# XuShenLZ/conflict_rez

Hardware: AMD Instinct MI355X
Metric: OBCA MPC-step solves/sec (4 vehicles, N=30) (higher is better)
Workload: dtype f64

## Files before the change

### conflict_rez_amd/csrc/cfz_engine.hip

```cpp

#include <hip/hip_runtime.h>
#include <stdio.h>
#include <string.h>

#include <algorithm>
#include <cstdio>
#include <cstdlib>
#include <unistd.h>
#include <cmath>
#include <string>
#include <tuple>
#include <vector>

#include "../../include/confrez_hip.h"
#include "cfz_solver.inl"
#include "cfz_audit.inl"
#include "cfz_disturb.inl"
#include "cfz_comm.inl"
#include "cfz_common.h"

thread_local std::string cfz_g_err;

namespace {

// ... 53 lines not shown
__global__ void loop_prep(int S, int V, int N, int T, const double *ref_table, const int32_t *table_of, const int32_t *kidx,
                          const double *pred, const double *state, double *x0, double *ref, double *nbr,
                          double *zu, int r, const int32_t *xperm, const int32_t *xrank, cfz::DisturbArgs dz, int step, cfz::CommArgs cm) {
  const long tid = (long)blockIdx.x * blockDim.x + threadIdx.x;
  if (tid >= (long)(xperm ? S : S * V) * N) return;
  const int k = (int)(tid % N);
  int b = (int)(tid / N);
  if (xperm) b = b * V + xperm[b * V + r];
  const int s = b / V, v = b - s * V;
  if (k < 5) x0[b * 5 + k] = dz.sigma ? cfz::disturb_add(state[b * 5 + k], cfz::disturb_value(dz, s, v, step, k)) : state[b * 5 + k];
  prep_stage(b, k, N, T, V, v, ref_table + ((size_t)table_of[s] * V + v) * T * 7, kidx[s], pred + (size_t)b * 7 * N,
             pred + (size_t)s * V * 7 * N, 7, xrank ? xrank + (size_t)s * V : nullptr, r, cm, s, step, ref, nbr, zu);
}

__global__ void advance_clock(int S, int K, int32_t *kidx) {
  const int s = blockIdx.x * blockDim.x + threadIdx.x;
  if (s < S) kidx[s] += K;
}

__global__ void loop_post(int S, int V, int N, const KArgs *ka, const int32_t *status, const int32_t *iters, const double *zu,
                          double *pred, double *state, int32_t *kidx, double *rec, int32_t *rec_si, int r, const int32_t *xperm,
                          cfz::DisturbArgs dz, int step, int32_t *carry, double *msg, const KArgs *pool, const int32_t *problem_of) {
  int b = blockIdx.x * blockDim.x + threadIdx.x;
  if (b >= (xperm ? S : S * V)) return;
  if (xperm) b = b * V + xperm[b * V + r];
  double *pb = pred + (size_t)b * 7 * N;
  if (status[b] == 0) {
    for (int i = 0; i < 7 * N; ++i) pb[i] = zu[(size_t)b * 7 * N + i];
  } else {
    for (int c = 0; c < 7; ++c)
      for (int k = 0; k + 1 < N; ++k) pb[c * N + k] = pb[c * N + k + 1];
  }
  if (msg)
    for (int i = 0; i < 7 * N; ++i) msg[(size_t)b * 7 * N + i] = pb[i];
  double z[5], out[5];
  for (int i = 0; i < 5; ++i) z[i] = state[b * 5 + i];
  double a0 = pb[5 * N], w0 = pb[6 * N];
  const int s = b / V, v = b - s * V;
  const cfz::KSpec &sp = (pool ? pool + problem_of[s] : ka)->sp;
  if (dz.sigma) {
    a0 = cfz::disturb_clip(cfz::disturb_add(a0, cfz::disturb_value(dz, s, v, step, 5)), sp.bounds[8], sp.bounds[9]);
    w0 = cfz::disturb_clip(cfz::disturb_add(w0, cfz::disturb_value(dz, s, v, step, 6)), sp.bounds[10], sp.bounds[11]);
  }
  cfz::rk4_step<false>(z, a0, w0, sp.dt, sp.wb, kPlantSubsteps, out, nullptr);
  if (dz.sigma)
    for (int i = 0; i < 5; ++i) out[i] = cfz::disturb_add(out[i], cfz::disturb_value(dz, s, v, step, 7 + i));
  for (int i = 0; i < 5; ++i) state[b * 5 + i] = out[i];
  if (kidx && (xperm ? r == V - 1 : b % V == 0)) kidx[b / V] += 1;
  if (carry) carry[b] = status[b] == 0;
  if (rec) {
    double *r = rec + (size_t)b * 7;
    for (int i = 0; i < 5; ++i) r[i] = out[i];
    r[5] = a0; r[6] = w0;
    rec_si[b] = status[b]; rec_si[S * V + b] = iters[b];
  }
}

__global__ void vs_prep(int S, int V, int n_own, int N, int T, const int32_t *own, const double *table, const int32_t *k0, int t,
                        const double *allpred, const double *pred, const double *state, double *x0, double *ref, double *nbr,
                        double *zu) {
  const long tid = (long)blockIdx.x * blockDim.x + threadIdx.x;
  if (tid >= (long)S * n_own * N) return;
  const int k = (int)(tid % N);
  const int b = (int)(tid / N);
  const int s = b / n_own, o = b - s * n_own;
  if (k < 5) x0[b * 5 + k] = state[b * 5 + k];
  prep_stage(b, k, N, T, V, own[o], table + (size_t)o * T * 7, k0[s] + t, pred + (size_t)b * 7 * N, allpred + (size_t)s * V * 3 * N, 3,
             nullptr, 0, cfz::comm_none(), s, t, ref, nbr, zu);
}

__global__ __launch_bounds__(1024) void order_by_iters(int B, const int32_t *iters, int32_t *order) {
  __shared__ int hist[1024];
  const int t = threadIdx.x;
  hist[t] = 0;
  __syncthreads();
  for (int b = t; b < B; b += 1024) atomicAdd(&hist[1023 - min(iters[b], 1023)], 1);
  __syncthreads();
  if (t == 0) { int acc = 0; for (int i = 0; i < 1024; ++i) { const int c = hist[i]; hist[i] = acc; acc += c; } }
  __syncthreads();
  for (int b = t; b < B; b += 1024) order[atomicAdd(&hist[1023 - min(iters[b], 1023)], 1)] = b;
}

#ifdef CFZ_LOOP_TRACE
constexpr int kLoopTraceWords = 5;
__device__ long long *cfz_loop_trace_buf;
#define CFZ_MARK(c) do { if (threadIdx.x == 0) __hip_atomic_store(&ctrl[4 + blockIdx.x], (c), __ATOMIC_RELAXED, __HIP_MEMORY_SCOPE_AGENT); } while (0)
#define CFZ_ITEM_STAMP(w, flag) do { if (threadIdx.x == 0) { long long *cfz_r = cfz_loop_trace_buf + ((size_t)t * B + b) * kLoopTraceWords;      \
                                                        cfz_r[w] = (long long)wall_clock64(); if ((w) == 0) cfz_r[4] = 1 + (flag); } } while (0)
#else
#define CFZ_MARK(c) do { } while (0)
#define CFZ_ITEM_STAMP(w, flag) do { } while (0)
#endif
#define CFZ_LOOP_ARGS const KArgs *__restrict__ ka, int S, int V, int K, int T, const double *ref_table, const int32_t *table_of,        \
                      const int32_t *kidx0, int t_base, double *pred, double *state, double *scratch, int32_t *qbuf, int32_t *ctrl,       \
                      int32_t *done, int32_t *status, int32_t *iters, double *stats, int32_t *iter_sum, double *wst, int wst_stride,     \
                      int prio_lag, int prio_tail, double *rec, int32_t *rec_si
__global__ __launch_bounds__(cfz::kNL, CFZ_WAVES_PER_SIMD) void loop_kernel(CFZ_LOOP_ARGS) {
  constexpr bool kSeq = false, kDist = false, kComm = false, kPool = false;
  const KArgs *const pool = nullptr; const int32_t *const problem_of = nullptr; constexpr bool dz_clip = true;
  const cfz::CommArgs cm = cfz::comm_none();
  const int32_t *const xperm = nullptr, *const xrank = nullptr;
  const cfz::DisturbArgs dz = cfz::disturb_none();
  const int step0 = 0;
#include "cfz_loop_body.inl"
}

__global__ __launch_bounds__(cfz::kNL, CFZ_WAVES_PER_SIMD) void loop_kernel_seq(CFZ_LOOP_ARGS, const int32_t *xperm, const int32_t *xrank) {
  constexpr bool kSeq = true, kDist = false, kComm = false, kPool = false;
  const KArgs *const pool = nullptr; const int32_t *const problem_of = nullptr; constexpr bool dz_clip = true;
  const cfz::CommArgs cm = cfz::comm_none();
  const cfz::DisturbArgs dz = cfz::disturb_none();
  const int step0 = 0;
#include "cfz_loop_body.inl"
}

__global__ __launch_bounds__(cfz::kNL, CFZ_WAVES_PER_SIMD) void loop_kernel_dist(CFZ_LOOP_ARGS, cfz::DisturbArgs dz, int step0) {
  constexpr bool kSeq = false, kDist = true, kComm = false, kPool = false;
  const KArgs *const pool = nullptr; const int32_t *const problem_of = nullptr; constexpr bool dz_clip = true;
  const cfz::CommArgs cm = cfz::comm_none();
  const int32_t *const xperm = nullptr, *const xrank = nullptr;
#include "cfz_loop_body.inl"
}

__global__ __launch_bounds__(cfz::kNL, CFZ_WAVES_PER_SIMD) void loop_kernel_seq_dist(CFZ_LOOP_ARGS, const int32_t *xperm,
                                                                 const int32_t *xrank, cfz::DisturbArgs dz, int step0) {
  constexpr bool kSeq = true, kDist = true, kComm = false, kPool = false;
  const KArgs *const pool = nullptr; const int32_t *const problem_of = nullptr; constexpr bool dz_clip = true;
  const cfz::CommArgs cm = cfz::comm_none();
#include "cfz_loop_body.inl"
}

__global__ __launch_bounds__(cfz::kNL, CFZ_WAVES_PER_SIMD) void loop_kernel_comm(CFZ_LOOP_ARGS, cfz::DisturbArgs dz, int step0,
                                                             cfz::CommArgs cm) {
  constexpr bool kSeq = false, kDist = true, kComm = true, kPool = false;
  const KArgs *const pool = nullptr; const int32_t *const problem_of = nullptr; constexpr bool dz_clip = true;
  const int32_t *const xperm = nullptr, *const xrank = nullptr;
#include "cfz_loop_body.inl"
}

__global__ __launch_bounds__(cfz::kNL, CFZ_WAVES_PER_SIMD) void loop_kernel_seq_comm(CFZ_LOOP_ARGS, const int32_t *xperm,
                                                                 const int32_t *xrank, cfz::DisturbArgs dz, int step0, cfz::CommArgs cm) {
  constexpr bool kSeq = true, kDist = true, kComm = true, kPool = false;
  const KArgs *const pool = nullptr; const int32_t *const problem_of = nullptr; constexpr bool dz_clip = true;
#include "cfz_loop_body.inl"
}

__global__ __launch_bounds__(cfz::kNL, CFZ_WAVES_PER_SIMD) void loop_kernel_pool(CFZ_LOOP_ARGS, cfz::DisturbArgs dz, int step0,
                                                             const KArgs *__restrict__ pool, const int32_t *__restrict__ problem_of, int dz_clip) {
  constexpr bool kSeq = false, kDist = true, kComm = false, kPool = true;
  const cfz::CommArgs cm = cfz::comm_none();
  const int32_t *const xperm = nullptr, *const xrank = nullptr;
#include "cfz_loop_body.inl"
}

__global__ __launch_bounds__(cfz::kNL, CFZ_WAVES_PER_SIMD) void loop_kernel_seq_pool(CFZ_LOOP_ARGS, const int32_t *xperm, const int32_t *xrank,
                                                                 cfz::DisturbArgs dz, int step0, const KArgs *__restrict__ pool,
                                                                 const int32_t *__restrict__ problem_of, int dz_clip) {
  constexpr bool kSeq = true, kDist = true, kComm = false, kPool = true;
  const cfz::CommArgs cm = cfz::comm_none();
#include "cfz_loop_body.inl"
}

__global__ __launch_bounds__(cfz::kNL, CFZ_WAVES_PER_SIMD) void loop_kernel_pool_comm(CFZ_LOOP_ARGS, cfz::DisturbArgs dz, int step0, cfz::CommArgs cm,
                                                                  const KArgs *__restrict__ pool, const int32_t *__restrict__ problem_of, int dz_clip) {
  constexpr bool kSeq = false, kDist = true, kComm = true, kPool = true;
  const int32_t *const xperm = nullptr, *const xrank = nullptr;
#include "cfz_loop_body.inl"
}

__global__ __launch_bounds__(cfz::kNL, CFZ_WAVES_PER_SIMD) void loop_kernel_seq_pool_comm(CFZ_LOOP_ARGS, const int32_t *xperm, const int32_t *xrank,
                                                                      cfz::DisturbArgs dz, int step0, cfz::CommArgs cm,
                                                                      const KArgs *__restrict__ pool, const int32_t *__restrict__ problem_of, int dz_clip) {
  constexpr bool kSeq = true, kDist = true, kComm = true, kPool = true;
#include "cfz_loop_body.inl"
}
#undef CFZ_LOOP_ARGS

constexpr int kLoopPrioLag = 0, kLoopPrioTailDiv = 0;
#ifdef CFZ_LOOP_TRACE
long long *g_loop_trace_dev = nullptr; size_t g_loop_trace_items = 0; int g_loop_trace_grid = 0;
#endif
struct LoopVariant { const void *fn; bool seq, dist, comm, pool; };
const LoopVariant kLoopVariants[10] = {
    {(const void *)loop_kernel, false, false, false, false},          {(const void *)loop_kernel_seq, true, false, false, false},
    {(const void *)loop_kernel_dist, false, true, false, false},      {(const void *)loop_kernel_seq_dist, true, true, false, false},
    {(const void *)loop_kernel_comm, false, true, true, false},       {(const void *)loop_kernel_seq_comm, true, true, true, false},
    {(const void *)loop_kernel_pool, false, true, false, true},       {(const void *)loop_kernel_seq_pool, true, true, false, true},
    {(const void *)loop_kernel_pool_comm, false, true, true, true},   {(const void *)loop_kernel_seq_pool_comm, true, true, true, true}};

int loop_variant(bool seq, bool dz_on, bool cm_on, bool pb_on) {
  const bool dist = dz_on || cm_on || pb_on;
  for (int i = 0; i < 10; ++i) {
    const LoopVariant &v = kLoopVariants[i];
    if (v.seq == seq && v.dist == dist && v.comm == cm_on && v.pool == pb_on) return i;
  }
  return -1;
}

__global__ void comm_fill(cfz::CommArgs cm, int S, int V, int tau0, long n, int32_t *delivered) {
  const long i = (long)blockIdx.x * blockDim.x + threadIdx.x;
  if (i >= n) return;
  const int u = (int)(i % V), v = (int)((i / V) % V), s = (int)((i / ((long)V * V)) % S), k = (int)(i / ((long)V * V * S));
  delivered[i] = u == v ? 1 : (cfz::comm_delivered(cm.seed, cm.stream[s], v, u, tau0 + k, cm.p_drop[s]) ? 1 : 0);
}

__global__ void disturb_fill(cfz::DisturbArgs dz, int S, int V, int t0, long n, double *d) {
  const long i = (long)blockIdx.x * blockDim.x + threadIdx.x;
  if (i >= n) return;
  const int c = (int)(i % cfz::kDisturbN);
  const long b = i / cfz::kDisturbN;
  const int v = (int)(b % V), s = (int)((b / V) % S), k = (int)(b / ((long)V * S));
  d[i] = cfz::disturb_value(dz, s, v, t0 + k, c);
}

__device__ inline void point_segment(double qx, double qy, double ax, double ay, double bx, double by, double &dist2, double &nx, double &ny) {
  const double ex = bx - ax, ey = by - ay, wx = qx - ax, wy = qy - ay;
  double t = (wx * ex + wy * ey) / (ex * ex + ey * ey);
  t = fmin(fmax(t, 0.0), 1.0);
  nx = wx - t * ex; ny = wy - t * ey;
  dist2 = nx * nx + ny * ny;
}

__device__ inline bool polygon_gap(const double PV[4][2], const double QV[4][2], double &nx, double &ny, double &dist) {
  double best = INFINITY, bx = 0.0, by = 0.0;
  for (int v = 0; v < 4; ++v)
    for (int e = 0; e < 4; ++e) {
      double d2, ux, uy;
      point_segment(QV[v][0], QV[v][1], PV[e][0], PV[e][1], PV[(e + 1) & 3][0], PV[(e + 1) & 3][1], d2, ux, uy);
      if (d2 < best) { best = d2; bx = ux; by = uy; }
      point_segment(PV[v][0], PV[v][1], QV[e][0], QV[e][1], QV[(e + 1) & 3][0], QV[(e + 1) & 3][1], d2, ux, uy);
      if (d2 < best) { best = d2; bx = -ux; by = -uy; }
    }
  dist = sqrt(best);
  if (!(dist > 1e-12)) return false;
  nx = bx / dist; ny = by / dist;
  return true;
}

__device__ inline void cone_duals(const double A[4][2], const double b[4], const double V[4][2], double nx, double ny, double lam[4]) {
  int v = 0; double sup = -INFINITY;
  for (int i = 0; i < 4; ++i) { const double h = nx * V[i][0] + ny * V[i][1]; if (h > sup) { sup = h; v = i; } }
  int i0 = 0, i1 = 1; double r0 = INFINITY, r1 = INFINITY;
  for (int i = 0; i < 4; ++i) {
    const double r = fabs(A[i][0] * V[v][0] + A[i][1] * V[v][1] - b[i]);
    if (r < r0) { r1 = r0; i1 = i0; r0 = r; i0 = i; } else if (r < r1) { r1 = r; i1 = i; }
  }
  const int ia = i0 < i1 ? i0 : i1, ib = i0 < i1 ? i1 : i0;
  const double det = A[ia][0] * A[ib][1] - A[ib][0] * A[ia][1];
  for (int i = 0; i < 4; ++i) lam[i] = 0.0;
  lam[ia] = fmax((A[ib][1] * nx - A[ib][0] * ny) / det, 0.0);
  lam[ib] = fmax((-A[ia][1] * nx + A[ia][0] * ny) / det, 0.0);
}

__global__ void dual_ws_kernel(const cfz::KSpec sp, int n, const double *poses, double *l, double *mu_out, double *d) {
  const int tid = blockIdx.x * blockDim.x + threadIdx.x;
  const int no = sp.n_obs;
  if (tid >= n * no) return;
  const int k = tid / no, j = tid - k * no;
  double A[4][2], b[4], V[4][2];
  for (int i = 0; i < 4; ++i) {
    A[i][0] = sp.A_obs[j][i][0]; A[i][1] = sp.A_obs[j][i][1]; b[i] = sp.b_obs[j][i];
// ... 97 lines not shown
  if (i >= n) return;
  double s, c;
  sincos(traj[i * 7 + 2], &s, &c);
  cs[i * 2] = c; cs[i * 2 + 1] = s;
}

__global__ __launch_bounds__(64) void audit_kernel(const KArgs *__restrict__ ka, int K, int S, int V, const double *traj,
                                                   const double *cs, const double *goal, const cfz::AuditPoly *obs_in, double il0, double il1,
                                                   double pos_tol, double psi_tol, double v_tol, double *clear, int32_t *where,
                                                   int32_t *first_contact, int32_t *arrive) {
  __shared__ cfz::AuditPoly obs[cfz::kMaxObs];
  const int s = blockIdx.x, lane = threadIdx.x;
  const int no = ka->sp.n_obs;
  if (lane < no) obs[lane] = obs_in[lane];
  double g[4];
  for (int i = 0; i < 4; ++i) g[i] = ka->sp.g[i];
  const double il[2] = {il0, il1};
  __syncthreads();
  cfz::AuditAcc acc;
  cfz::audit_lane(acc, lane, 64, K, V, traj + (size_t)s * V * 7, (long)S * V * 7, goal + (size_t)s * V * 3, cs + (size_t)s * V * 2, no,
                  obs, g, il, pos_tol, psi_tol, v_tol);
  for (int off = 32; off > 0; off >>= 1) {
    cfz::AuditAcc o;
    o.vv = __shfl_xor(acc.vv, off, 64); o.vv_t = __shfl_xor(acc.vv_t, off, 64); o.vv_u = __shfl_xor(acc.vv_u, off, 64);
    o.vv_w = __shfl_xor(acc.vv_w, off, 64);
    o.vo = __shfl_xor(acc.vo, off, 64); o.vo_t = __shfl_xor(acc.vo_t, off, 64); o.vo_v = __shfl_xor(acc.vo_v, off, 64);
    o.vo_j = __shfl_xor(acc.vo_j, off, 64);
    o.first = __shfl_xor(acc.first, off, 64);
    for (int v = 0; v < cfz::kAuditMaxV; ++v) o.arrive[v] = __shfl_xor(acc.arrive[v], off, 64);
    cfz::audit_merge(acc, o);
  }
  if (lane == 0) cfz::audit_store(acc, V, clear + (size_t)s * 2, where + (size_t)s * 6, first_contact + s, arrive + (size_t)s * V);
}

}

struct cfz_handle {
  int device = 0, max_batch = 0;
  cfz::KSpec ks;
  cfz::Lay lay;
  cfz_spec spec0;
  cfz_options opt0;
  size_t lds_bytes = 0;
  int blocks_per_cu = 0;
  hipStream_t stream = nullptr;
  hipEvent_t ev0 = nullptr, ev1 = nullptr;
  float last_ms = 0.f;
  double *obs_tab = nullptr;
  KArgs *kargs = nullptr;
  double *wst = nullptr;
  int32_t *carry = nullptr, *slots = nullptr;
  int32_t *stage_host = nullptr;
  hipEvent_t ev_stage = nullptr;
  int wst_stride = 0, carry_duals = 1;
  bool carry_set = false, slots_set = false, ms_pending = false;
  const int32_t *carry_ext = nullptr;
  double *x0 = nullptr, *ref = nullptr, *nbr = nullptr, *zu = nullptr, *stats = nullptr;
  int32_t *status = nullptr, *iters = nullptr;
  double *l = nullptr, *m = nullptr, *lam_ij = nullptr, *lam_ji = nullptr, *s = nullptr;
  struct Loop {
    int S = 0, T = 0, P = 0;
    double *ref_table = nullptr, *pred = nullptr, *state = nullptr;
    int32_t *kidx = nullptr, *order = nullptr, *table_of = nullptr;
    bool have_order = false;
    int32_t *xperm = nullptr, *xrank = nullptr, *xlist = nullptr;
    std::vector<int32_t> xperm_host;
    double *rec = nullptr;
    int32_t *rec_si = nullptr;
    int rec_cap = 0, rec_used = 0;
    void *dz_buf = nullptr, *dz_zero = nullptr;
    uint64_t dz_seed = 0;
    bool dz_on = false;
    void *cm_buf = nullptr;
    double *cm_ring = nullptr;
    uint64_t cm_seed = 0;
    int cm_max_age = 0, cm_compensate = 0, cm_tau_on = 0, cm_ring_slots = 0;
    bool cm_on = false;
    KArgs *pb_pool = nullptr;
    int32_t *pb_of = nullptr;
    int pb_cap = 0;
    bool pb_on = false;
    double *pred2 = nullptr, *scratch = nullptr;
    int32_t *queue = nullptr, *ctrl = nullptr, *done = nullptr, *iter_sum = nullptr;
    int queue_cap = 0, grid_blocks = 0, steps_done = 0;
  } lp;
  long last_iter_sum = 0, last_converged = 0, last_status[6] = {0, 0, 0, 0, 0, 0};
  CfzArena arena;
};

namespace {

int launch_solve(cfz_handle *h, int B, const double *x0, const double *ref, const double *nbr, double *zu,
                 int32_t *status, int32_t *iters, double *stats, bool duals, hipStream_t st,
                 const int32_t *order = nullptr, int carry_all = 0, int grid = 0, bool pool = false) {
  DualPtrs du = {nullptr, nullptr, nullptr, nullptr, nullptr};
  if (duals) du = {h->l, h->m, h->lam_ij, h->lam_ji, h->s};
  if ((h->carry_set || h->slots_set) && st != h->stream) HIP_OK(hipStreamWaitEvent(st, h->ev_stage, 0));
  HIP_OK(hipEventRecord(h->ev0, st));
  const int32_t *carry = h->carry_ext ? h->carry_ext : (h->carry_set ? h->carry : nullptr);
  auto launch = [&](auto kernel, auto... tail) {
    hipLaunchKernelGGL(kernel, dim3(grid ? grid : B), dim3(cfz::kNL), h->lds_bytes, st, h->kargs, B, x0, ref, nbr, zu, status, iters, stats, du,
                       order, h->carry_duals ? h->wst : nullptr, h->wst_stride, carry, carry_all, h->slots_set ? h->slots : nullptr, tail...);
  };
  if (pool)
    launch(solve_kernel_pool, h->lp.pb_pool, h->lp.pb_of, h->ks.n_nbr + 1);
  else
    launch(solve_kernel);
  h->carry_set = false; h->slots_set = false; h->carry_ext = nullptr;
  h->ms_pending = true;
  HIP_OK(hipGetLastError());
  HIP_OK(hipEventRecord(h->ev1, st));
  return 0;
}

int create_fill(cfz_handle *h, const cfz_spec *spec, const cfz_options *opt);
void loop_release(cfz_handle *h);

int spec_shape_ok(const cfz_spec *spec) {
  if (spec->N < 2 || spec->N > CFZ_MAX_N) return fail("N out of range");
  if (spec->n_obs < 0 || spec->n_obs > CFZ_MAX_OBS || spec->n_nbr < 0 || spec->n_nbr > CFZ_MAX_NBR)
    return fail("n_obs / n_nbr out of range");
  if (spec->N > cfz::kMaxN) return fail("N exceeds the four-lanes-per-stage kernel");
  return 0;
}

int options_ok(const cfz_options *opt) {
  if (opt->filter_cap < 1 || opt->filter_cap > 32) return fail("filter_cap must be in 1..32");
  if (opt->restoration < 0 || !(opt->reg_dual_rows >= 0.0) || !(opt->resto_first >= 0.0)) return fail("restoration, reg_dual_rows, resto_first must not be negative");
  return 0;
}

int fill_kspec(cfz::KSpec &k, const cfz_spec *spec, const cfz_options *opt) {
  memset(&k, 0, sizeof k);
  k.N = spec->N; k.n_obs = spec->n_obs; k.n_nbr = spec->n_nbr; k.rk_substeps = spec->rk_substeps;
  k.max_iter = opt->max_iter; k.max_backtrack = opt->max_backtrack; k.filter_cap = opt->filter_cap;
  k.dt = spec->dt; k.wb = spec->wb; k.dmin = spec->dmin;
  memcpy(k.g, spec->g, sizeof k.g); memcpy(k.bounds, spec->bounds, sizeof k.bounds);
  memcpy(k.weights, spec->weights, sizeof k.weights);
  for (int j = 0; j < spec->n_obs; ++j) {
    memcpy(k.A_obs[j], spec->A_obs[j], sizeof k.A_obs[j]); memcpy(k.b_obs[j], spec->b_obs[j], sizeof k.b_obs[j]);
    if (!quad_vertices(spec->A_obs[j], spec->b_obs[j], k.V_obs[j])) return fail("obstacle is not a bounded quadrilateral");
  }
  k.tol = opt->tol; k.constr_viol_tol = opt->constr_viol_tol; k.dual_inf_tol = opt->dual_inf_tol;
  k.compl_inf_tol = opt->compl_inf_tol; k.mu_init = opt->mu_init; k.kappa_eps = opt->kappa_eps;
  k.kappa_mu = opt->kappa_mu; k.theta_mu = opt->theta_mu; k.tau_min = opt->tau_min; k.bound_push = opt->bound_push;
  k.bound_frac = opt->bound_frac; k.s_max = opt->s_max; k.kappa_sigma = opt->kappa_sigma; k.eta_phi = opt->eta_phi;
  k.gamma_theta = opt->gamma_theta; k.gamma_phi = opt->gamma_phi; k.delta_sw = opt->delta_sw;
  k.s_theta = opt->s_theta; k.s_phi = opt->s_phi; k.reg_primal = opt->reg_primal;
  k.stall_iters = opt->stall_iters; k.stall_kappa = opt->stall_kappa; k.row_curvature = opt->row_curvature; k.vv_rows = opt->vv_rows; k.shift_after = opt->shift_after; k.resto = opt->restoration; k.stag_win = opt->shift_stagnation; k.err_stall = opt->err_stall_iters; k.carry_shift = opt->carry_shift ? 1 : 0; k.pad_ks = 0; k.warm_push = opt->warm_push; k.reg_dual_rows = opt->reg_dual_rows; k.resto_first = opt->resto_first;
  return 0;
}

int check(cfz_handle *h, int B) {
  if (!h) return fail("null handle");
  if (B < 1 || B > h->max_batch) return fail("batch size out of range");
  HIP_OK(hipSetDevice(h->device));
  return 0;
}

}

extern "C" {

const char *cfz_last_error(void) { return cfz_g_err.c_str(); }

#ifndef CFZ_SRC_HASH
// ... 267 lines not shown
                     d_state, nullptr, nullptr, nullptr, 0, nullptr, cfz::disturb_none(), 0, d_carry, nullptr, nullptr, nullptr);
  HIP_OK(hipGetLastError());
  return 0;
}

int cfz_dual_ws(cfz_handle *h, int n, const double *poses, double *l, double *m, double *d) {
  if (!h) return fail("null handle");
  if (n < 1 || !poses || !l || !m) return fail("bad argument");
  HIP_OK(hipSetDevice(h->device));
  const size_t no = h->ks.n_obs;
  if (no == 0) return 0;
  double *dp = nullptr, *dl = nullptr, *dm = nullptr, *dd = nullptr;
  if (arena_reset(h->arena)) return -1;
  ARENA_ALLOC(h->arena, dp, (size_t)n * 3 * 8); ARENA_ALLOC(h->arena, dl, (size_t)n * 4 * no * 8);
  ARENA_ALLOC(h->arena, dm, (size_t)n * 4 * no * 8); ARENA_ALLOC(h->arena, dd, (size_t)n * no * 8);
  HIP_OK(hipMemcpyAsync(dp, poses, (size_t)n * 3 * 8, hipMemcpyHostToDevice, h->stream));
  const int nt = n * (int)no;
  hipLaunchKernelGGL(dual_ws_kernel, dim3((nt + 127) / 128), dim3(128), 0, h->stream, h->ks, n, dp, dl, dm, dd);
  HIP_OK(hipGetLastError());
  HIP_OK(hipMemcpyAsync(l, dl, (size_t)n * 4 * no * 8, hipMemcpyDeviceToHost, h->stream));
  HIP_OK(hipMemcpyAsync(m, dm, (size_t)n * 4 * no * 8, hipMemcpyDeviceToHost, h->stream));
  if (d) HIP_OK(hipMemcpyAsync(d, dd, (size_t)n * no * 8, hipMemcpyDeviceToHost, h->stream));
  HIP_OK(hipStreamSynchronize(h->stream));
  return 0;
}

int cfz_joint_dual_ws(cfz_handle *h, int n, const double *poses_this, const double *poses_other, double *lam, double *mu,
                      double *s, double *d) {
  if (!h) return fail("null handle");
  if (n < 1 || !poses_this || !poses_other || !lam || !mu || !s) return fail("bad argument");
  HIP_OK(hipSetDevice(h->device));
  double *dpa = nullptr, *dpb = nullptr, *dout = nullptr;
  if (arena_reset(h->arena)) return -1;
  ARENA_ALLOC(h->arena, dpa, (size_t)n * 3 * 8); ARENA_ALLOC(h->arena, dpb, (size_t)n * 3 * 8); ARENA_ALLOC(h->arena, dout, (size_t)n * 11 * 8);
  HIP_OK(hipMemcpyAsync(dpa, poses_this, (size_t)n * 3 * 8, hipMemcpyHostToDevice, h->stream));
  HIP_OK(hipMemcpyAsync(dpb, poses_other, (size_t)n * 3 * 8, hipMemcpyHostToDevice, h->stream));
  double *dl = dout, *dm = dout + (size_t)n * 4, *ds = dout + (size_t)n * 8, *dd = dout + (size_t)n * 10;
  hipLaunchKernelGGL(joint_dual_ws_kernel, dim3((n + 127) / 128), dim3(128), 0, h->stream, h->ks, n, dpa, dpb, dl, dm, ds, dd);
  HIP_OK(hipGetLastError());
  HIP_OK(hipMemcpyAsync(lam, dl, (size_t)n * 4 * 8, hipMemcpyDeviceToHost, h->stream)); HIP_OK(hipMemcpyAsync(mu, dm, (size_t)n * 4 * 8, hipMemcpyDeviceToHost, h->stream));
  HIP_OK(hipMemcpyAsync(s, ds, (size_t)n * 2 * 8, hipMemcpyDeviceToHost, h->stream));
  if (d) HIP_OK(hipMemcpyAsync(d, dd, (size_t)n * 8, hipMemcpyDeviceToHost, h->stream));
  HIP_OK(hipStreamSynchronize(h->stream));
  return 0;
}

}

namespace {
template <class T> void dev_free(T *&p) {
  if (p) (void)hipFree(p);
  p = nullptr;
}

void record_free(cfz_handle *h) {
  dev_free(h->lp.rec); dev_free(h->lp.rec_si);
  h->lp.rec_cap = h->lp.rec_used = 0;
}

void exchange_free(cfz_handle *h) {
  dev_free(h->lp.xperm); dev_free(h->lp.xrank); dev_free(h->lp.xlist);
  h->lp.xperm_host.clear();
}

void disturb_free(cfz_handle *h) {
  dev_free(h->lp.dz_buf);
  h->lp.dz_on = false; h->lp.dz_seed = 0;
}

void comm_free(cfz_handle *h) {
  dev_free(h->lp.cm_buf); dev_free(h->lp.cm_ring);
  h->lp.cm_on = false; h->lp.cm_ring_slots = 0;
}

void problems_free(cfz_handle *h) {
  dev_free(h->lp.pb_pool); dev_free(h->lp.pb_of);
  h->lp.pb_on = false; h->lp.pb_cap = 0;
}

void loop_release(cfz_handle *h) {
  record_free(h); exchange_free(h); disturb_free(h); comm_free(h); problems_free(h);
  dev_free(h->lp.dz_zero);
  dev_free(h->lp.ref_table); dev_free(h->lp.table_of); dev_free(h->lp.pred); dev_free(h->lp.state); dev_free(h->lp.kidx); dev_free(h->lp.order);
  dev_free(h->lp.pred2); dev_free(h->lp.scratch); dev_free(h->lp.queue); dev_free(h->lp.ctrl); dev_free(h->lp.done); dev_free(h->lp.iter_sum);
  h->lp = cfz_handle::Loop();
}

cfz::DisturbArgs disturb_args(const cfz_handle *h, bool zero_if_off = false) {
  if (!h->lp.dz_on && !zero_if_off) return cfz::disturb_none();
  const double *f = static_cast<const double *>(h->lp.dz_on ? h->lp.dz_buf : h->lp.dz_zero);
  return {h->lp.dz_on ? h->lp.dz_seed : 0, f, f + cfz::kDisturbN, reinterpret_cast<const uint32_t *>(f + cfz::kDisturbN + h->lp.S)};
}

cfz::CommArgs comm_args(const cfz_handle *h) {
  if (!h->lp.cm_on) return cfz::comm_none();
  const double *f = static_cast<const double *>(h->lp.cm_buf);
  const size_t S = (size_t)h->lp.S;
  return {h->lp.cm_seed, f, reinterpret_cast<const uint32_t *>(f + S), h->lp.cm_ring, h->lp.cm_max_age, h->lp.cm_compensate, h->lp.cm_tau_on,
          S * (h->ks.n_nbr + 1) * 7 * h->ks.N};
}

int loop_ready(cfz_handle *h, bool drain = false) {
  if (!h || !h->lp.pred) return fail("cfz_loop_init has not been called");
  HIP_OK(hipSetDevice(h->device));
  if (drain) HIP_OK(hipStreamSynchronize(h->stream));
  return 0;
}

int upload_setting(cfz_handle *h, void *&buf, const std::vector<double> &f, const uint32_t *stream) {
  std::vector<uint32_t> id((size_t)h->lp.S);
  for (size_t s = 0; s < id.size(); ++s) id[s] = stream ? stream[s] : (uint32_t)s;
  if (!buf) HIP_OK(hipMalloc(&buf, f.size() * 8 + id.size() * 4));
  HIP_OK(hipMemcpy(buf, f.data(), f.size() * 8, hipMemcpyHostToDevice));
  HIP_OK(hipMemcpy(static_cast<char *>(buf) + f.size() * 8, id.data(), id.size() * 4, hipMemcpyHostToDevice));
  return 0;
}

double *comm_message(const cfz_handle *h, int tau) {
  return h->lp.cm_ring + (size_t)cfz::comm_slot(tau, h->lp.cm_max_age) * comm_args(h).slot_stride;
}

int record_room(cfz_handle *h, int steps) {
  if (h->lp.rec_cap && h->lp.rec_used + steps > h->lp.rec_cap) return fail("the step(s) would overflow the record (cfz_loop_record)");
  return 0;
}

void record_slice(const cfz_handle *h, double *&rec, int32_t *&rec_si) {
  const size_t B = (size_t)h->lp.S * (h->ks.n_nbr + 1);
  rec = h->lp.rec ? h->lp.rec + (size_t)h->lp.rec_used * B * 7 : nullptr;
  rec_si = h->lp.rec ? h->lp.rec_si + (size_t)h->lp.rec_used * 2 * B : nullptr;
}

int loop_round(cfz_handle *h, int r, int n_inst, const int32_t *dispatch, const int32_t *xperm, const int32_t *xrank) {
  const int V = h->ks.n_nbr + 1, N = h->ks.N, S = h->lp.S;
  double *rec; int32_t *rec_si;
  record_slice(h, rec, rec_si);
  const cfz::DisturbArgs dz = disturb_args(h);
  const cfz::CommArgs cm = comm_args(h);
  const long nt = (long)n_inst * N;
  hipLaunchKernelGGL(loop_prep, dim3((unsigned)((nt + 255) / 256)), dim3(256), 0, h->stream, S, V, N, h->lp.T, h->lp.ref_table,
                     h->lp.table_of, h->lp.kidx, h->lp.pred, h->lp.state, h->x0, h->ref, h->nbr, h->zu, r, xperm, xrank, dz, h->lp.steps_done, cm);
  HIP_OK(hipGetLastError());
  const bool pool = h->lp.pb_on;
  if (launch_solve(h, S * V, h->x0, h->ref, h->nbr, h->zu, h->status, h->iters, h->stats, false, h->stream, dispatch, 1, n_inst, pool)) return -1;
  hipLaunchKernelGGL(loop_post, dim3((unsigned)((n_inst + 63) / 64)), dim3(64), 0, h->stream, S, V, N, h->kargs, h->status, h->iters, h->zu,
                     h->lp.pred, h->lp.state, h->lp.kidx, rec, rec_si, r, xperm, dz, h->lp.steps_done, nullptr,
                     h->lp.cm_on ? comm_message(h, h->lp.steps_done) : nullptr, pool ? h->lp.pb_pool : nullptr, pool ? h->lp.pb_of : nullptr);
  HIP_OK(hipGetLastError());
  return 0;
}

int audit_launch(cfz_handle *h, int K, int S, int V, const double *d_traj, const double *d_goal, double pos_tol, double psi_tol,
                 double v_tol, double *clear, int32_t *where, int32_t *first_contact, int32_t *arrive) {
  const int no = h->ks.n_obs;
  std::vector<cfz::AuditPoly> ob((size_t)std::max(no, 1));
  for (int j = 0; j < no; ++j) {
    memcpy(ob[j].v, h->ks.V_obs[j], sizeof ob[j].v);
    cfz::audit_poly_prepare(ob[j]);
  }
  const double *g = h->ks.g;
  double *dc = nullptr, *dcs = nullptr;
  int32_t *di = nullptr;
  cfz::AuditPoly *dob = nullptr;
  const long n = (long)K * S * V;
  ARENA_ALLOC(h->arena, dc, (size_t)S * 2 * 8); ARENA_ALLOC(h->arena, di, (size_t)S * (7 + V) * 4);
  ARENA_ALLOC(h->arena, dcs, (size_t)n * 2 * 8);
  ARENA_ALLOC(h->arena, dob, ob.size() * sizeof(cfz::AuditPoly));
// ... 230 lines not shown
int cfz_loop_set_problems(cfz_handle *h, int P, const cfz_spec *specs, const cfz_options *opts, const int32_t *problem_of) {
  if (loop_ready(h, true)) return -1;
  if (P < 0) return fail("P must not be negative");
  if (P == 0 || !specs) { h->lp.pb_on = false; return 0; }
  if (!problem_of) return fail("null problem_of");
  const int S = h->lp.S;
  for (int s = 0; s < S; ++s)
    if (problem_of[s] < 0 || problem_of[s] >= P) return fail("problem_of[s] outside [0, P)");
  std::vector<KArgs> pool((size_t)P);
  for (int p = 0; p < P; ++p) {
    const cfz_options *o = opts ? &opts[p] : &h->opt0;
    if (cfz_problem_check(&h->spec0, &h->opt0, &specs[p], o)) { cfz_g_err = "problem " + std::to_string(p) + ": " + cfz_g_err; return -1; }
    if (fill_kspec(pool[p].sp, &specs[p], o)) return -1;
    pool[p].sp.obs_tab = h->obs_tab;
    pool[p].dv = cfz::derive(pool[p].sp); pool[p].L = h->lay;
  }
  KArgs *d = nullptr;
  int32_t *of = nullptr;
  hipError_t e = hipMalloc(&d, (size_t)P * sizeof(KArgs));
  if (e == hipSuccess) e = hipMalloc(&of, (size_t)S * 4);
  if (e == hipSuccess) e = hipMemcpy(d, pool.data(), (size_t)P * sizeof(KArgs), hipMemcpyHostToDevice);
  if (e == hipSuccess) e = hipMemcpy(of, problem_of, (size_t)S * 4, hipMemcpyHostToDevice);
  if (e != hipSuccess) { dev_free(d); dev_free(of); return fail("cfz_loop_set_problems: device copy of the pool", e); }
  dev_free(h->lp.pb_pool); dev_free(h->lp.pb_of);
  h->lp.pb_pool = d; h->lp.pb_of = of; h->lp.pb_cap = P;
  h->lp.pb_on = true;
  return 0;
}

int cfz_loop_comm(cfz_handle *h, int tau0, int K, int32_t *delivered) {
  if (loop_ready(h)) return -1;
  if (!h->lp.cm_on) return fail("no lossy exchange is set (cfz_loop_set_comm)");
  if (tau0 < 0 || K < 1 || !delivered) return fail("tau0 must not be negative, K must be positive and delivered not NULL");
  const int S = h->lp.S, V = h->ks.n_nbr + 1;
  const size_t n = (size_t)K * S * V * V;
  if (n > ((size_t)1 << 31)) return fail("window too large");
  if (arena_reset(h->arena)) return -1;
  int32_t *dd = nullptr;
  ARENA_ALLOC(h->arena, dd, n * 4);
  hipLaunchKernelGGL(comm_fill, dim3((unsigned)((n + 255) / 256)), dim3(256), 0, h->stream, comm_args(h), S, V, tau0, (long)n, dd);
  HIP_OK(hipGetLastError());
  HIP_OK(hipMemcpyAsync(delivered, dd, n * 4, hipMemcpyDeviceToHost, h->stream));
  HIP_OK(hipStreamSynchronize(h->stream));
  return 0;
}

int cfz_loop_step(cfz_handle *h) {
  if (loop_ready(h) || record_room(h, 1)) return -1;
  const int V = h->ks.n_nbr + 1, S = h->lp.S, B = S * V;
  float total_ms = 0.f;
  if (h->lp.xperm) {
    for (int r = 0; r < V; ++r) {
      if (r > 0) {
        HIP_OK(hipEventSynchronize(h->ev1));
        float ms = 0.f;
        HIP_OK(hipEventElapsedTime(&ms, h->ev0, h->ev1)); total_ms += ms;
      }
      if (loop_round(h, r, S, h->lp.xlist + (size_t)r * S, h->lp.xperm, h->lp.xrank)) return -1;
    }
    h->lp.have_order = false;
  } else {
    if (loop_round(h, 0, B, h->lp.have_order ? h->lp.order : nullptr, nullptr, nullptr)) return -1;
    hipLaunchKernelGGL(order_by_iters, dim3(1), dim3(1024), 0, h->stream, B, h->iters, h->lp.order);
    HIP_OK(hipGetLastError());
    h->lp.have_order = true;
  }
  if (h->lp.rec) h->lp.rec_used += 1;
  h->lp.steps_done += 1;
  HIP_OK(hipStreamSynchronize(h->stream));
  float ms = 0.f;
  HIP_OK(hipEventElapsedTime(&ms, h->ev0, h->ev1));
  h->last_ms = total_ms + ms;
  h->ms_pending = false;
  return 0;
}

int cfz_loop_run(cfz_handle *h, int K) {
  if (loop_ready(h)) return -1;
  if (K < 1) return fail("K must be positive");
  if (record_room(h, K)) return -1;
  const int V = h->ks.n_nbr + 1, N = h->ks.N, S = h->lp.S, B = S * V;
  const size_t total = (size_t)B * K;
  if (total > (size_t)1 << 30) return fail("too many work items");
  int ncu = 0;
  HIP_OK(hipDeviceGetAttribute(&ncu, hipDeviceAttributeMultiprocessorCount, h->device));
  int per_cu = 0;
  const bool seq = h->lp.xperm != nullptr, comm = h->lp.cm_on;
  const int variant = loop_variant(seq, h->lp.dz_on, comm, h->lp.pb_on);
  if (variant < 0) return fail("no persistent kernel for this setting");
  const LoopVariant &var = kLoopVariants[variant];
  HIP_OK(hipOccupancyMaxActiveBlocksPerMultiprocessor(&per_cu, var.fn, cfz::kNL, h->lds_bytes));
  per_cu = std::min(per_cu, h->blocks_per_cu);
  if (per_cu < 1) return fail("loop kernel does not fit on a CU");
  if (const char *cap = std::getenv("CFZ_LOOP_BLOCKS_PER_CU")) per_cu = std::max(1, std::min(per_cu, std::atoi(cap)));
  const int grid = std::min(seq ? S : B, per_cu * ncu);
  const size_t per_block = 5 + 3 * (size_t)N + (size_t)h->ks.n_nbr * 3 * N + 7 * (size_t)N;
  if (!h->lp.pred2) {
    HIP_OK(hipMalloc(&h->lp.pred2, (size_t)2 * B * 7 * N * 8)); HIP_OK(hipMalloc(&h->lp.ctrl, (4 + 1024) * 4));
    HIP_OK(hipMalloc(&h->lp.done, (size_t)S * 4)); HIP_OK(hipMalloc(&h->lp.iter_sum, 32));
  }
  if (h->lp.grid_blocks < grid) {
    if (h->lp.scratch) (void)hipFree(h->lp.scratch);
    HIP_OK(hipMalloc(&h->lp.scratch, (size_t)grid * per_block * 8)); h->lp.grid_blocks = grid;
  }
  const size_t qwords = 2 * (size_t)K + total;
  if ((size_t)h->lp.queue_cap < qwords) {
    if (h->lp.queue) (void)hipFree(h->lp.queue);
    HIP_OK(hipMalloc(&h->lp.queue, qwords * 4)); h->lp.queue_cap = (int)qwords;
  }
  if (!comm) HIP_OK(hipMemcpyAsync(h->lp.pred2, h->lp.pred, (size_t)B * 7 * N * 8, hipMemcpyDeviceToDevice, h->stream));
  HIP_OK(hipMemsetAsync(h->lp.queue, 0, 2 * (size_t)K * 4, h->stream));
  HIP_OK(hipMemsetAsync(h->lp.queue + 2 * K, 0xff, total * 4, h->stream));
  {
    const int n0 = seq ? S : B;
    std::vector<int32_t> first(n0);
    for (int i = 0; i < n0; ++i) first[i] = seq ? i * V + h->lp.xperm_host[(size_t)i * V] : i;
    HIP_OK(hipMemcpyAsync(h->lp.queue + 2 * K, first.data(), (size_t)n0 * 4, hipMemcpyHostToDevice, h->stream));
    HIP_OK(hipMemcpyAsync(h->lp.queue + K, &n0, 4, hipMemcpyHostToDevice, h->stream));
    const int32_t ctrl0[4] = {0, 0, 0, 0};
    HIP_OK(hipMemcpyAsync(h->lp.ctrl, ctrl0, sizeof ctrl0, hipMemcpyHostToDevice, h->stream));
    HIP_OK(hipMemsetAsync(h->lp.done, 0, (size_t)S * 4, h->stream));
    HIP_OK(hipMemsetAsync(h->lp.iter_sum, 0, 32, h->stream));
    HIP_OK(hipStreamSynchronize(h->stream));
  }
  HIP_OK(hipEventRecord(h->ev0, h->stream));
  double *rec; int32_t *rec_si;
  record_slice(h, rec, rec_si);
  const int prio_lag = std::getenv("CFZ_LOOP_PRIO_LAG") ? std::atoi(std::getenv("CFZ_LOOP_PRIO_LAG")) : kLoopPrioLag;
  const int prio_tail = std::getenv("CFZ_LOOP_PRIO_TAIL") ? std::max(0, std::atoi(std::getenv("CFZ_LOOP_PRIO_TAIL")))
                                                          : (kLoopPrioTailDiv > 0 ? std::max(V, B / kLoopPrioTailDiv) : 0);
#ifdef CFZ_LOOP_TRACE
  {
    static long long *trace_dev = nullptr; static size_t trace_cap = 0;
    if (trace_cap < total) {
      if (trace_dev) (void)hipFree(trace_dev);
      HIP_OK(hipMalloc(&trace_dev, total * kLoopTraceWords * 8)); trace_cap = total;
      HIP_OK(hipMemcpyToSymbol(HIP_SYMBOL(cfz_loop_trace_buf), &trace_dev, sizeof trace_dev));
    }
    HIP_OK(hipMemsetAsync(trace_dev, 0, total * kLoopTraceWords * 8, h->stream));
    g_loop_trace_dev = trace_dev; g_loop_trace_items = total; g_loop_trace_grid = grid;
  }
#endif
  const auto xo = std::make_tuple((const int32_t *)h->lp.xperm, (const int32_t *)h->lp.xrank);
  const auto dz = std::make_tuple(disturb_args(h, true), h->lp.steps_done);
  const auto cm = std::make_tuple(comm_args(h));
  const auto pb = std::make_tuple((const KArgs *)h->lp.pb_pool, (const int32_t *)h->lp.pb_of, h->lp.dz_on ? 1 : 0);
  auto launch = [&](auto kernel, const auto &...groups) {
    if ((const void *)kernel != var.fn) return fail("cfz_loop_run: the launch chain and kLoopVariants name different kernels");
    std::apply([&](auto... tail) {
      hipLaunchKernelGGL(kernel, dim3(grid), dim3(cfz::kNL), h->lds_bytes, h->stream, h->kargs, S, V, K, h->lp.T, h->lp.ref_table, h->lp.table_of,
                         h->lp.kidx, 0, h->lp.pred2, h->lp.state, h->lp.scratch, h->lp.queue, h->lp.ctrl, h->lp.done, h->status, h->iters, h->stats,
                         h->lp.iter_sum, h->carry_duals ? h->wst : nullptr, h->wst_stride, prio_lag, prio_tail, rec, rec_si, tail...);
    }, std::tuple_cat(groups...));
    return 0;
  };
  int bad = 0;
  switch (variant) {
    case 0: bad = launch(loop_kernel); break;
    case 1: bad = launch(loop_kernel_seq, xo); break;
    case 2: bad = launch(loop_kernel_dist, dz); break;
    case 3: bad = launch(loop_kernel_seq_dist, xo, dz); break;
    case 4: bad = launch(loop_kernel_comm, dz, cm); break;
    case 5: bad = launch(loop_kernel_seq_comm, xo, dz, cm); break;
    case 6: bad = launch(loop_kernel_pool, dz, pb); break;
    case 7: bad = launch(loop_kernel_seq_pool, xo, dz, pb); break;
    case 8: bad = launch(loop_kernel_pool_comm, dz, cm, pb); break;
    case 9: bad = launch(loop_kernel_seq_pool_comm, xo, dz, cm, pb); break;
  }
  if (bad) return -1;
  HIP_OK(hipGetLastError());
  if (h->lp.rec) h->lp.rec_used += K;
  h->lp.steps_done += K;
  HIP_OK(hipEventRecord(h->ev1, h->stream));
  HIP_OK(hipMemcpyAsync(h->lp.pred, comm ? comm_message(h, h->lp.steps_done - 1) : h->lp.pred2 + (size_t)(K & 1) * B * 7 * N, (size_t)B * 7 * N * 8, hipMemcpyDeviceToDevice, h->stream));
  hipLaunchKernelGGL(advance_clock, dim3((S + 255) / 256), dim3(256), 0, h->stream, S, K, h->lp.kidx);
  HIP_OK(hipGetLastError());
  if (const char *dbg = std::getenv("CFZ_LOOP_WATCHDOG")) {
    const double limit_s = std::atof(dbg) > 0 ? std::atof(dbg) : 10.0;
    hipStream_t s2; HIP_OK(hipStreamCreateWithFlags(&s2, hipStreamNonBlocking));
    int32_t last_head = -1; double stalled = 0.0;
    while (hipEventQuery(h->ev1) == hipErrorNotReady) {
      usleep(100000);
      int32_t c[4] = {0, 0, 0, 0};
      HIP_OK(hipMemcpyAsync(c, h->lp.ctrl, sizeof c, hipMemcpyDeviceToHost, s2)); HIP_OK(hipStreamSynchronize(s2));
      std::fprintf(stderr, "[cfz watchdog] lowest open iteration %d, completed %d of %zu, err %d (grid %d)", c[0], c[1], total, c[2], grid);
#ifdef CFZ_LOOP_TRACE
      int32_t mk[8];
      HIP_OK(hipMemcpyAsync(mk, h->lp.ctrl + 4, sizeof mk, hipMemcpyDeviceToHost, s2)); HIP_OK(hipStreamSynchronize(s2));
      for (int i = 0; i < 8 && i < grid; ++i) std::fprintf(stderr, " m%d=%d", i, mk[i]);
#endif
      std::fprintf(stderr, "\n");
      stalled = (c[1] == last_head) ? stalled + 0.1 : 0.0; last_head = c[1];
      if (stalled > limit_s) {
        const int32_t one = 1;
        HIP_OK(hipMemcpyAsync(h->lp.ctrl + 2, &one, 4, hipMemcpyHostToDevice, s2)); HIP_OK(hipStreamSynchronize(s2));
        stalled = -1e9;
      }
    }
    (void)hipStreamDestroy(s2);
  }
  HIP_OK(hipStreamSynchronize(h->stream));
  HIP_OK(hipEventElapsedTime(&h->last_ms, h->ev0, h->ev1));
  h->ms_pending = false;
  int32_t ctrl[4] = {0, 0, 0, 0}, isum[8] = {0, 0, 0, 0, 0, 0, 0, 0};
  HIP_OK(hipMemcpy(ctrl, h->lp.ctrl, sizeof ctrl, hipMemcpyDeviceToHost));
  HIP_OK(hipMemcpy(isum, h->lp.iter_sum, 32, hipMemcpyDeviceToHost));
  h->last_iter_sum = isum[0]; h->last_converged = isum[1];
  for (int i = 0; i < 6; ++i) h->last_status[i] = isum[2 + i];
  h->lp.have_order = false;
  if (ctrl[2]) return fail("persistent loop kernel timed out waiting for a work item");
  return 0;
}

#ifdef CFZ_LOOP_TRACE
extern "C" int cfz_loop_trace_read(long long *out, long n) {
  if (!out || !g_loop_trace_dev || (size_t)n != g_loop_trace_items) return fail("cfz_loop_trace_read: no trace of that many items");
  HIP_OK(hipMemcpy(out, g_loop_trace_dev, g_loop_trace_items * kLoopTraceWords * 8, hipMemcpyDeviceToHost));
  return g_loop_trace_grid;
}
#endif

long cfz_loop_last_iterations(const cfz_handle *h) { return h ? h->last_iter_sum : -1; }
long cfz_loop_last_converged(const cfz_handle *h) { return h ? h->last_converged : -1; }
int cfz_loop_last_status_counts(const cfz_handle *h, long counts[6]) {
  if (!h || !counts) return fail("null argument");
  for (int i = 0; i < 6; ++i) counts[i] = h->last_status[i];
  return 0;
}

int cfz_loop_get(cfz_handle *h, double *state, double *pred, int32_t *status, int32_t *iters) {
  if (loop_ready(h)) return -1;
  const size_t B = (size_t)h->lp.S * (h->ks.n_nbr + 1), N = h->ks.N;
  if (state) HIP_OK(hipMemcpy(state, h->lp.state, B * 5 * 8, hipMemcpyDeviceToHost));
  if (pred) HIP_OK(hipMemcpy(pred, h->lp.pred, B * 7 * N * 8, hipMemcpyDeviceToHost));
  if (status) HIP_OK(hipMemcpy(status, h->status, B * 4, hipMemcpyDeviceToHost));
  if (iters) HIP_OK(hipMemcpy(iters, h->iters, B * 4, hipMemcpyDeviceToHost));
  return 0;
}

}
```

Baseline: 5.416 million.

## Add hardware-placement keyed clear table plumbing to persistent loop kernel

Adds a device table keyed by XCC and CU hardware ID, and passes it to the persistent loop kernels along with domain, yield and prefer polling parameters that can be set from the environment. The intent is to let work items be claimed with awareness of the chiplet or CU they run on, which should improve cache locality and reduce cross-die traffic. The trace records gain fields for placement key and poll counts. The default domain is 0, so the scheme is probably inactive unless enabled, and it adds kernel arguments and a per-setup memset.

Result: slower. 5.330 million (-1.6%).

```diff
diff --git a/conflict_rez_amd/csrc/cfz_engine.hip b/conflict_rez_amd/csrc/cfz_engine.hip
--- a/conflict_rez_amd/csrc/cfz_engine.hip
+++ b/conflict_rez_amd/csrc/cfz_engine.hip
@@ -159,19 +159,32 @@
 }
 
 #ifdef CFZ_LOOP_TRACE
-constexpr int kLoopTraceWords = 5;
+constexpr int kLoopTraceWords = 7;
 __device__ long long *cfz_loop_trace_buf;
 #define CFZ_MARK(c) do { if (threadIdx.x == 0) __hip_atomic_store(&ctrl[4 + blockIdx.x], (c), __ATOMIC_RELAXED, __HIP_MEMORY_SCOPE_AGENT); } while (0)
 #define CFZ_ITEM_STAMP(w, flag) do { if (threadIdx.x == 0) { long long *cfz_r = cfz_loop_trace_buf + ((size_t)t * B + b) * kLoopTraceWords;      \
                                                         cfz_r[w] = (long long)wall_clock64(); if ((w) == 0) cfz_r[4] = 1 + (flag); } } while (0)
+#define CFZ_ITEM_PLACE(key, seen, polls) do { if (threadIdx.x == 0) { long long *cfz_r = cfz_loop_trace_buf + ((size_t)t * B + b) * kLoopTraceWords;   \
+                                                        cfz_r[5] = (long long)(key) | (long long)blockIdx.x << 16;                                \
+                                                        cfz_r[6] = (long long)(seen) | (long long)(polls) << 32; } } while (0)
 #else
 #define CFZ_MARK(c) do { } while (0)
 #define CFZ_ITEM_STAMP(w, flag) do { } while (0)
+#define CFZ_ITEM_PLACE(key, seen, polls) do { } while (0)
 #endif
+constexpr int kLoopClearKeys = 1 << 12;
+constexpr int kLoopClearMaxPolls = 1 << 12;
+__device__ __forceinline__ int loop_place_key() {
+  uint32_t xcc, hw;
+  asm volatile("s_getreg_b32 %0, hwreg(HW_REG_XCC_ID, 0, 4)" : "=s"(xcc));
+  asm volatile("s_getreg_b32 %0, hwreg(HW_REG_HW_ID, 8, 8)" : "=s"(hw));
+  return (int)((xcc & 15u) << 8 | (hw & 255u));
+}
 #define CFZ_LOOP_ARGS const KArgs *__restrict__ ka, int S, int V, int K, int T, const double *ref_table, const int32_t *table_of,        \
                       const int32_t *kidx0, int t_base, double *pred, double *state, double *scratch, int32_t *qbuf, int32_t *ctrl,       \
                       int32_t *done, int32_t *status, int32_t *iters, double *stats, int32_t *iter_sum, double *wst, int wst_stride,     \
-                      int prio_lag, int prio_tail, double *rec, int32_t *rec_si
+                      int prio_lag, int prio_tail, int32_t *clear_tab, int clear_dom, int clear_yield, int clear_prefer, double *rec,  \
+                      int32_t *rec_si
 __global__ __launch_bounds__(cfz::kNL, CFZ_WAVES_PER_SIMD) void loop_kernel(CFZ_LOOP_ARGS) {
   constexpr bool kSeq = false, kDist = false, kComm = false, kPool = false;
   const KArgs *const pool = nullptr; const int32_t *const problem_of = nullptr; constexpr bool dz_clip = true;
@@ -254,6 +267,7 @@
 #undef CFZ_LOOP_ARGS
 
 constexpr int kLoopPrioLag = 0, kLoopPrioTailDiv = 0;
+constexpr int kLoopClearDomain = 0, kLoopClearYield = 256, kLoopClearPrefer = 2;
 #ifdef CFZ_LOOP_TRACE
 long long *g_loop_trace_dev = nullptr; size_t g_loop_trace_items = 0; int g_loop_trace_grid = 0;
 #endif
@@ -517,6 +531,7 @@
     bool pb_on = false;
     double *pred2 = nullptr, *scratch = nullptr;
     int32_t *queue = nullptr, *ctrl = nullptr, *done = nullptr, *iter_sum = nullptr;
+    int32_t *clear_tab = nullptr;
     int queue_cap = 0, grid_blocks = 0, steps_done = 0;
   } lp;
   long last_iter_sum = 0, last_converged = 0, last_status[6] = {0, 0, 0, 0, 0, 0};
@@ -950,7 +965,7 @@
   record_free(h); exchange_free(h); disturb_free(h); comm_free(h); problems_free(h);
   dev_free(h->lp.dz_zero);
   dev_free(h->lp.ref_table); dev_free(h->lp.table_of); dev_free(h->lp.pred); dev_free(h->lp.state); dev_free(h->lp.kidx); dev_free(h->lp.order);
-  dev_free(h->lp.pred2); dev_free(h->lp.scratch); dev_free(h->lp.queue); dev_free(h->lp.ctrl); dev_free(h->lp.done); dev_free(h->lp.iter_sum);
+  dev_free(h->lp.pred2); dev_free(h->lp.scratch); dev_free(h->lp.queue); dev_free(h->lp.ctrl); dev_free(h->lp.clear_tab); dev_free(h->lp.done); dev_free(h->lp.iter_sum);
   h->lp = cfz_handle::Loop();
 }
 
@@ -1347,6 +1362,13 @@
   const int V = h->ks.n_nbr + 1, N = h->ks.N, S = h->lp.S, B = S * V;
   const size_t total = (size_t)B * K;
   if (total > (size_t)1 << 30) return fail("too many work items");
+  const int clear_dom = std::getenv("CFZ_LOOP_CLEAR_DOMAIN") ? std::atoi(std::getenv("CFZ_LOOP_CLEAR_DOMAIN")) : kLoopClearDomain;
+  if (clear_dom != 0 && clear_dom != 1 && clear_dom != 2 && clear_dom != 9) return fail("CFZ_LOOP_CLEAR_DOMAIN must be 0, 1, 2 or 9");
+  const auto polls = [](const char *name, int builtin) {
+    const char *v = std::getenv(name);
+    return std::max(0, std::min(v ? std::atoi(v) : builtin, kLoopClearMaxPolls));
+  };
+  const int clear_yield = polls("CFZ_LOOP_CLEAR_YIELD", kLoopClearYield), clear_prefer = polls("CFZ_LOOP_CLEAR_PREFER", kLoopClearPrefer);
   int ncu = 0;
   HIP_OK(hipDeviceGetAttribute(&ncu, hipDeviceAttributeMultiprocessorCount, h->device));
   int per_cu = 0;
@@ -1362,6 +1384,7 @@
   const size_t per_block = 5 + 3 * (size_t)N + (size_t)h->ks.n_nbr * 3 * N + 7 * (size_t)N;
   if (!h->lp.pred2) {
     HIP_OK(hipMalloc(&h->lp.pred2, (size_t)2 * B * 7 * N * 8)); HIP_OK(hipMalloc(&h->lp.ctrl, (4 + 1024) * 4));
+    HIP_OK(hipMalloc(&h->lp.clear_tab, (size_t)2 * kLoopClearKeys * 4));
     HIP_OK(hipMalloc(&h->lp.done, (size_t)S * 4)); HIP_OK(hipMalloc(&h->lp.iter_sum, 32));
   }
   if (h->lp.grid_blocks < grid) {
@@ -1386,6 +1409,7 @@
     HIP_OK(hipMemcpyAsync(h->lp.ctrl, ctrl0, sizeof ctrl0, hipMemcpyHostToDevice, h->stream));
     HIP_OK(hipMemsetAsync(h->lp.done, 0, (size_t)S * 4, h->stream));
     HIP_OK(hipMemsetAsync(h->lp.iter_sum, 0, 32, h->stream));
+    HIP_OK(hipMemsetAsync(h->lp.clear_tab, 0, (size_t)2 * kLoopClearKeys * 4, h->stream));
     HIP_OK(hipStreamSynchronize(h->stream));
   }
   HIP_OK(hipEventRecord(h->ev0, h->stream));
@@ -1415,7 +1439,7 @@
     std::apply([&](auto... tail) {
       hipLaunchKernelGGL(kernel, dim3(grid), dim3(cfz::kNL), h->lds_bytes, h->stream, h->kargs, S, V, K, h->lp.T, h->lp.ref_table, h->lp.table_of,
                          h->lp.kidx, 0, h->lp.pred2, h->lp.state, h->lp.scratch, h->lp.queue, h->lp.ctrl, h->lp.done, h->status, h->iters, h->stats,
-                         h->lp.iter_sum, h->carry_duals ? h->wst : nullptr, h->wst_stride, prio_lag, prio_tail, rec, rec_si, tail...);
+                         h->lp.iter_sum, h->carry_duals ? h->wst : nullptr, h->wst_stride, prio_lag, prio_tail, h->lp.clear_tab, clear_dom, clear_yield, clear_prefer, rec, rec_si, tail...);
     }, std::tuple_cat(groups...));
     return 0;
   };
@@ -1483,6 +1507,7 @@
   HIP_OK(hipMemcpy(out, g_loop_trace_dev, g_loop_trace_items * kLoopTraceWords * 8, hipMemcpyDeviceToHost));
   return g_loop_trace_grid;
 }
+extern "C" int cfz_loop_trace_words(void) { return kLoopTraceWords; }
 #endif
 
 long cfz_loop_last_iterations(const cfz_handle *h) { return h ? h->last_iter_sum : -1; }
```
